# akanimax/thr3ed_atom

Measured on AMD Instinct MI355X. Metric: ray-samples/sec (fwd+bwd) training step, 800x800 images @ 128^3 SH-2 ReLU field, higher is better.
Workload: dtype f32

## Files before the change

include/relu_field.h:

```cpp
#ifndef RELU_FIELD_H_
#define RELU_FIELD_H_

#include <stdint.h>

#ifdef __cplusplus
extern "C" {
#endif

#define RF_ABI_VERSION 4
#define RF_BRICK_4X8X8 488

enum {
  RF_OK = 0,
  RF_ERR_NULL_POINTER = -1,
  RF_ERR_BAD_SHAPE = -2,
  RF_ERR_UNSUPPORTED = -3,
  RF_ERR_LAUNCH = -4
};

enum {
  RF_DENSITY_RELU = 0,
  RF_DENSITY_SOFTPLUS = 1,
  RF_DENSITY_ABS = 2,
  RF_DENSITY_IDENTITY = 3
// ... 117 lines not shown
                            int32_t* hist_dev, void* stream);
int rf_scatter_records(const RFGrid* grid, const int16_t* keys_dev, const float* records_dev, int64_t capacity,
                       int32_t* cursor_dev, int32_t render_diffuse, float* records_sorted_dev, int32_t* hist_dev, int32_t num_keys,
                       void* stream);
int rf_expand_records(const RFGrid* grid, const float* records_dev, const int64_t* perm_dev, const int64_t* begin_dev,
                      int64_t capacity, int32_t render_diffuse, float* records_sorted_dev, void* stream);

int rf_brick_accumulate(const RFGrid* grid, int32_t brick_size, const RFBrickList* lists, int32_t num_lists,
                        float* grad_densities_dev, float* grad_features_dev, int32_t accumulate, void* stream);

typedef struct RFAdamState {
  float* param_first_dev;
  float* param_second_dev;
  float* exp_avg_first_dev;
  float* exp_avg_second_dev;
  float* exp_avg_sq_first_dev;
  float* exp_avg_sq_second_dev;
  float lr, beta1, beta2, eps;
  int32_t step;
} RFAdamState;

int rf_brick_accumulate_adam(const RFGrid* grid, int32_t brick_size, const RFBrickList* lists, int32_t num_lists,
                             const RFAdamState* adam, void* stream);

int rf_brick_accumulate_adam_mirror(const RFGrid* grid, int32_t brick_size, const RFBrickList* lists, int32_t num_lists,
                                    const RFAdamState* adam, float* mirror_densities_dev, float* mirror_features_dev, void* stream);

int rf_brick_accumulate_adam_range(const RFGrid* grid, int32_t brick_size, const RFBrickList* lists, int32_t num_lists,
                                   const RFAdamState* adam, int32_t first_brick, int32_t num_bricks, void* stream);

int64_t rf_brick_split_scratch_bytes(const RFGrid* grid, int32_t num_bricks, int32_t parts);
int rf_brick_accumulate_adam_split(const RFGrid* grid, int32_t brick_size, const RFBrickList* lists, int32_t num_lists,
                                   const RFAdamState* adam, int32_t first_brick, int32_t num_bricks, int32_t parts, void* scratch_dev,
                                   int64_t scratch_bytes, void* stream);

int rf_grid_query(const RFGrid* grid, const float* points_dev, int64_t num_points, float* out_dev, void* stream);

int rf_grid_query_backward(const RFGrid* grid, const float* points_dev, int64_t num_points,
                           const float* grad_out_dev, float* grad_densities_dev, float* grad_features_dev,
                           void* stream);

int rf_build_occupancy(const RFGrid* grid, float threshold, uint32_t* occupancy_dev, void* stream);

int rf_upsample_grid(const RFGrid* src, const RFGrid* dst, void* stream);

int rf_convert_grid(const RFGrid* src, const RFGrid* dst, void* stream);
// ... 79 lines not shown
```

thr3ed_atom_amd/_lib.py:

```python
import ctypes as C
import os
import subprocess
from typing import Optional

CSRC_DIR = os.path.join(os.path.dirname(os.path.abspath(__file__)), "csrc")
INCLUDE_DIR = os.path.join(os.path.dirname(os.path.dirname(os.path.abspath(__file__))), "include")
LIB_NAME = "librelu_field_hip.so"
LIB_PATH = os.environ.get("RF_LIB_PATH") or os.path.join(CSRC_DIR, LIB_NAME)
SOURCES = ["relu_field_kernels.hip", "mesh_kernels.hip"]
HIPCC_FLAGS = ["--offload-arch=gfx950", "-O3", "-std=c++17", "-ffp-contract=off", "-fPIC", "-shared"]

ABI_VERSION = 4

DENSITY_MODES = {"relu": 0, "softplus": 1, "abs": 2, "identity": 3}
LAYOUTS = {"reference": 0, "split": 1, "bricked": 2}
FLAG_WHITE_BKGD = 1
FLAG_RENDER_DIFFUSE = 2
FLAG_AABB_SAMPLING = 4
FLAG_OCCUPANCY_SKIP = 8
FLAG_JITTER_KEYED = 16
ERR_UNSUPPORTED = -3
STEP_FORWARD = 1
STEP_EMIT = 2
STEP_BRICKS = 4
# ... 4 lines not shown
STEP_DIFFUSE_CHAIN = 128
STEP_SPECULAR_FORWARD = 256

EXPORTED_SYMBOLS = [
    "rf_abi_version",
    "rf_abi_struct_size",
    "rf_error_string",
    "rf_cast_rays",
    "rf_cast_selected_rays",
    "rf_select_rays_and_pixels",
    "rf_ray_aabb_bounds",
    "rf_render_forward",
    "rf_frame_render_kernel",
    "rf_render_backward",
    "rf_render_backward_emit",
    "rf_expand_records",
    "rf_expanded_record_floats",
    "rf_bin_offsets",
    "rf_render_backward_emit_direct",
    "rf_scatter_records",
    "rf_brick_accumulate",
    "rf_brick_accumulate_adam",
    "rf_brick_accumulate_adam_mirror",
    "rf_brick_accumulate_adam_range",
    "rf_brick_accumulate_adam_split",
    "rf_brick_split_scratch_bytes",
    "rf_grid_query",
    "rf_grid_query_backward",
    "rf_build_occupancy",
    "rf_upsample_grid",
    "rf_convert_grid",
    "rf_l1_loss_grad",
    "rf_adam_step",
    "rf_train_step",
    "rf_render_forward_pair",
    "rf_l1_loss_grad_pair",
    "rf_bin_offsets_pair",
    "rf_render_backward_emit_direct_pair",
    "rf_mesh_tiles",
    "rf_mesh_count",
    "rf_mesh_emit",
]


class RFGrid(C.Structure):
    _fields_ = [
# ... 188 lines not shown
        C.POINTER(RFRayBatch),
        u32,
        C.POINTER(RFRenderOut),
        C.POINTER(RFRenderGrads),
        vp,
        vp,
        vp,
    ]
    lib.rf_render_backward_emit.argtypes = [
        C.POINTER(RFGrid), C.POINTER(RFRayBatch), u32, C.POINTER(RFRenderOut), C.POINTER(RFRenderGrads), i32, vp, vp, vp, vp,
    ]
    lib.rf_expand_records.argtypes = [C.POINTER(RFGrid), vp, vp, vp, i64, i32, vp, vp]
    lib.rf_expanded_record_floats.argtypes = [i32]
    lib.rf_expanded_record_floats.restype = i32
    lib.rf_bin_offsets.argtypes = [vp, i32, vp, vp, vp]
    lib.rf_render_backward_emit_direct.argtypes = [
        C.POINTER(RFGrid), C.POINTER(RFRayBatch), u32, C.POINTER(RFRenderOut), C.POINTER(RFRenderGrads), i32, vp, vp, vp, vp,
    ]
    lib.rf_scatter_records.argtypes = [C.POINTER(RFGrid), vp, vp, i64, vp, i32, vp, vp, i32, vp]
    lib.rf_brick_accumulate.argtypes = [C.POINTER(RFGrid), i32, C.POINTER(RFBrickList), i32, vp, vp, i32, vp]
    lib.rf_brick_accumulate_adam.argtypes = [C.POINTER(RFGrid), i32, C.POINTER(RFBrickList), i32, C.POINTER(RFAdamState), vp]
    lib.rf_brick_accumulate_adam_range.argtypes = [C.POINTER(RFGrid), i32, C.POINTER(RFBrickList), i32, C.POINTER(RFAdamState), i32, i32, vp]
    lib.rf_brick_accumulate_adam_mirror.argtypes = [C.POINTER(RFGrid), i32, C.POINTER(RFBrickList), i32, C.POINTER(RFAdamState), vp, vp, vp]
    lib.rf_brick_accumulate_adam_split.argtypes = [C.POINTER(RFGrid), i32, C.POINTER(RFBrickList), i32, C.POINTER(RFAdamState), i32, i32, i32, vp, i64, vp]
    lib.rf_brick_split_scratch_bytes.argtypes = [C.POINTER(RFGrid), i32, i32]
    lib.rf_train_step.argtypes = [C.POINTER(RFGrid), C.POINTER(RFTrainStep), vp]
    lib.rf_grid_query.argtypes = [C.POINTER(RFGrid), vp, i64, vp, vp]
    lib.rf_grid_query_backward.argtypes = [C.POINTER(RFGrid), vp, i64, vp, vp, vp, vp]
    lib.rf_upsample_grid.argtypes = [C.POINTER(RFGrid), C.POINTER(RFGrid), vp]
    lib.rf_convert_grid.argtypes = [C.POINTER(RFGrid), C.POINTER(RFGrid), vp]
    lib.rf_build_occupancy.argtypes = [C.POINTER(RFGrid), f32, vp, vp]
    lib.rf_l1_loss_grad.argtypes = [vp, vp, i64, f32, vp, vp, vp]
    lib.rf_adam_step.argtypes = [vp, vp, vp, vp, i64, f32, f32, f32, f32, i32, i32, vp]
    lib.rf_render_forward_pair.argtypes = [C.POINTER(RFGrid), C.POINTER(RFRayBatch), C.POINTER(u32), C.POINTER(RFRenderOut), vp]
    lib.rf_l1_loss_grad_pair.argtypes = [C.POINTER(vp), vp, i64, f32, C.POINTER(vp), vp, vp, vp]
    lib.rf_bin_offsets_pair.argtypes = [C.POINTER(vp), i32, C.POINTER(vp), C.POINTER(vp), vp]
    lib.rf_render_backward_emit_direct_pair.argtypes = [C.POINTER(RFGrid), C.POINTER(RFRayBatch), C.POINTER(u32), C.POINTER(RFPassScratch), vp]
    lib.rf_mesh_tiles.argtypes = [C.POINTER(RFGrid), i32]
    lib.rf_mesh_count.argtypes = [C.POINTER(RFGrid), i32, f32, vp, vp]
    lib.rf_mesh_emit.argtypes = [C.POINTER(RFGrid), i32, f32, vp, i64, i64, vp, vp, vp, vp, vp, vp]
    for name in EXPORTED_SYMBOLS:
        if name not in ("rf_error_string",):
            getattr(lib, name).restype = C.c_int64 if name in ("rf_brick_split_scratch_bytes", "rf_mesh_tiles") else C.c_int
    if lib.rf_abi_version() != ABI_VERSION:
        raise RuntimeError(f"{LIB_PATH}: ABI version {lib.rf_abi_version()} != {ABI_VERSION} (stale build? run __graft_entry__.build())")
    lib.rf_abi_struct_size.argtypes = [C.c_int]
# ... 16 lines not shown
```

thr3ed_atom_amd/csrc/relu_field_kernels.hip:

```cpp
#include <hip/hip_runtime.h>
#include <stdint.h>

#include <atomic>
#include <cstdlib>
#include <type_traits>

#include "relu_field.h"

namespace {

#ifndef RF_FWD_WAVES
#define RF_FWD_WAVES 4
#endif
#ifndef RF_EMIT_WAVES
#define RF_EMIT_WAVES 6
#endif
#ifndef RF_EMIT_G
#define RF_EMIT_G 2
#endif
constexpr int kWave = 64;
constexpr int kWavesPerBlock = 4;
constexpr int kBlock = kWave * kWavesPerBlock;
constexpr float kInfinity = 1e10f;
constexpr float kZeroPlus = 1e-10f;
// ... 108 lines not shown
    *p = v;
  }
}
template <bool NT>
__device__ __forceinline__ float4 load_f4(const float4* p) {
  if constexpr (NT) {
    const vf4 t = __builtin_nontemporal_load(reinterpret_cast<const vf4*>(p));
    return make_float4(t[0], t[1], t[2], t[3]);
  } else {
    return *p;
  }
}
#ifndef RF_NT_RECORD_STORE
#define RF_NT_RECORD_STORE 1
#endif
#ifndef RF_NT_CACHE_STORE
#define RF_NT_CACHE_STORE 1
#endif
#ifndef RF_NT_RECORD_LOAD
#define RF_NT_RECORD_LOAD 0
#endif
#ifndef RF_NT_CACHE_LOAD
#define RF_NT_CACHE_LOAD 1
#endif

__device__ __forceinline__ void wave_lds_fence() {
  __builtin_amdgcn_fence(__ATOMIC_RELEASE, "wavefront");
  __builtin_amdgcn_wave_barrier();
  __builtin_amdgcn_fence(__ATOMIC_ACQUIRE, "wavefront");
}

template <int CTRL, int ROW_MASK>
__device__ __forceinline__ float dpp_move(float old, float src) {
  return __builtin_bit_cast(float, __builtin_amdgcn_update_dpp(__builtin_bit_cast(int, old), __builtin_bit_cast(int, src),
                                                               CTRL, ROW_MASK, 0xf, false));
}
constexpr int kDppRowShr1 = 0x111, kDppRowShr2 = 0x112, kDppRowShr4 = 0x114, kDppRowShr8 = 0x118;
constexpr int kDppRowBcast15 = 0x142, kDppRowBcast31 = 0x143, kDppWaveShr1 = 0x138, kDppWaveShl1 = 0x130;

__device__ __forceinline__ void wave_incl_scan_trans(float& e, float& a) {
  auto step = [&](auto ctrl_tag, auto mask_tag) {
    constexpr int CTRL = decltype(ctrl_tag)::value, MASK = decltype(mask_tag)::value;
    const float ep = dpp_move<CTRL, MASK>(1.0f, e), ap = dpp_move<CTRL, MASK>(0.0f, a);
    a = __builtin_fmaf(a, ep, ap);
    e = e * ep;
  };
// ... 1871 lines not shown
  const int B = ONE_ROUND ? 8 : (1 << a.shift);
  const int SY = brick_row_stride(B, C), SX = brick_slab_stride(B, C);
  const int tid = threadIdx.x;
  const bool split = g.layout == RF_LAYOUT_SPLIT;
  if (split && (C & 3) == 0 && (g.dstride & 3) == 0 && (C == 4 || (g.fstride & 3) == 0)) {
    constexpr int QN = C / 4;
    constexpr int QR = QN > 1 ? QN - 1 : 1;
    const int nq = (BX == 4 ? 4 : B) * B * B * QN;
    auto quad_of = [&](int i, int& fx, int& fy, int& fz, int& qd) -> bool {
      const int col = (i >> a.shift) / QN, r = i - col * (B * QN);
      const bool first = r < B;
      fz = first ? r : (r - B) / QR;
      qd = first ? 0 : 1 + (r - B) - fz * QR;
      fx = col >> a.shift;
      fy = col & (B - 1);
      return i < nq && X0 + fx < g.X && Y0 + fy < g.Y && Z0 + fz < g.Z;
    };
    if constexpr (ADAM) {
      constexpr int U = (QN == 7) ? 4 : 1;
      const AdamArgs& ad = a.adam;
      if constexpr (ONE_ROUND) {
        unsigned int bo[QN];
        int lds_at[QN];
        float4 p4[QN];
        vf4 m4[QN], v4[QN];
#pragma unroll
        for (int u = 0; u < QN; ++u) {
          int fx, fy, fz, qd;
          if (u == 0) {
            fx = tid >> 6;
            fy = (tid >> 3) & 7;
            fz = tid & 7;
            qd = 0;
          } else {
            const int j = (u - 1) * TH + tid, col = j / 48, r = j - col * 48;
            fz = r / 6;
            qd = 1 + r - 6 * fz;
            fx = col >> 3;
            fy = col & 7;
          }
          const bool ok = X0 + fx < g.X && Y0 + fy < g.Y && Z0 + fz < g.Z;
          const unsigned int lin = ok ? node_lin(g, X0 + fx, Y0 + fy, Z0 + fz) : 0u;
          const unsigned int o = u == 0 ? __umul24(lin, (unsigned)g.dstride) : __umul24(lin, (unsigned)g.fstride) + 4u * (unsigned)(qd - 1);
          bo[u] = ok ? o * 4u : 0xffffffffu;
          lds_at[u] = fx * SX + fy * SY + fz * CS + 4 * qd;
        }
#pragma unroll
        for (int u = 0; u < QN; ++u) {
          if (bo[u] != 0xffffffffu) {
            const char* pb = reinterpret_cast<const char*>(u == 0 ? ad.p1 : ad.p2);
            const char* mb = reinterpret_cast<const char*>(u == 0 ? ad.m1 : ad.m2);
            const char* vb = reinterpret_cast<const char*>(u == 0 ? ad.v1 : ad.v2);
            p4[u] = *reinterpret_cast<const float4*>(pb + bo[u]);
            m4[u] = __builtin_nontemporal_load(reinterpret_cast<const vf4*>(mb + bo[u]));
            v4[u] = __builtin_nontemporal_load(reinterpret_cast<const vf4*>(vb + bo[u]));
          }
        }
#pragma unroll
        for (int u = 0; u < QN; ++u) {
          if (bo[u] == 0xffffffffu) continue;
          const float4 gq = any ? *reinterpret_cast<const float4*>(&acc[lds_at[u]]) : make_float4(0.f, 0.f, 0.f, 0.f);
          float gg[4] = {gq.x, gq.y, gq.z, gq.w};
          float pn[4] = {p4[u].x, p4[u].y, p4[u].z, p4[u].w};
          if (u == 0 && g.mode == RF_DENSITY_ABS) {
            const float dv = pn[0] * g.rho;
            gg[0] = (dv > 0.f) ? gg[0] : ((dv < 0.f) ? -gg[0] : 0.0f);
          }
          vf4 mn, vn;
#pragma unroll
          for (int c = 0; c < 4; ++c) {
            float mm = m4[u][c], vv = v4[u][c];
            adam_update(pn[c], mm, vv, gg[c], ad.step, ad.b1, ad.b2, ad.eps, ad.inv_bc2_sqrt);
            mn[c] = mm;
            vn[c] = vv;
          }
          char* pb = reinterpret_cast<char*>(u == 0 ? ad.p1 : ad.p2);
          char* mb = reinterpret_cast<char*>(u == 0 ? ad.m1 : ad.m2);
          char* vb = reinterpret_cast<char*>(u == 0 ? ad.v1 : ad.v2);
          *reinterpret_cast<float4*>(pb + bo[u]) = make_float4(pn[0], pn[1], pn[2], pn[3]);
          __builtin_nontemporal_store(mn, reinterpret_cast<vf4*>(mb + bo[u]));
          __builtin_nontemporal_store(vn, reinterpret_cast<vf4*>(vb + bo[u]));
          if constexpr (MIRROR) *reinterpret_cast<float4*>(const_cast<float*>(&acc[lds_at[u]])) = make_float4(pn[0], pn[1], pn[2], pn[3]);
        }
        if constexpr (MIRROR) {
          __syncthreads();
          constexpr int F = 3 * K, FQ = 2 * F, CQ = FQ + 2;
          for (int i = tid; i < 32 * CQ; i += TH) {
            const int col = i / CQ, r = i - col * CQ;
            const int fx = col >> 3, fy = col & 7;
            const float* img = acc + fx * SX + fy * SY;
            const unsigned int lin0 = node_lin(g, X0 + fx, Y0 + fy, Z0);
            float v[4];
            if (r < FQ) {
#pragma unroll
              for (int t = 0; t < 4; ++t) {
                const int e = 4 * r + t;
                const int nz = e / F, f = e - nz * F;
                const int colour = f / K, k = f - colour * K;
                v[t] = img[nz * CS + (k == 0 ? 1 + colour : 4 + colour * (K - 1) + (k - 1))];
              }
              *reinterpret_cast<float4*>(gfeat + (size_t)(__umul24(lin0, (unsigned)F) + 4u * (unsigned)r)) = make_float4(v[0], v[1], v[2], v[3]);
            } else {
              const int z0 = 4 * (r - FQ);
#pragma unroll
              for (int t = 0; t < 4; ++t) v[t] = img[(z0 + t) * CS];
              *reinterpret_cast<float4*>(gdens + (size_t)(lin0 + (unsigned)z0)) = make_float4(v[0], v[1], v[2], v[3]);
// ... 536 lines not shown
      const unsigned long long* other = images + (long long)j * pairs;
      float2* own = reinterpret_cast<float2*>(acc);
      for (int i = tid; i < pairs; i += TH) {
        const unsigned long long o = __hip_atomic_load(other + i, __ATOMIC_RELAXED, __HIP_MEMORY_SCOPE_AGENT);
        float2 v = any ? own[i] : make_float2(0.f, 0.f);
        v.x += __uint_as_float((uint32_t)o);
        v.y += __uint_as_float((uint32_t)(o >> 32));
        own[i] = v;
      }
      any = true;
      __syncthreads();
    }
    if (tid <= parts) state[tid] = 0;
    __syncthreads();
  }
#if defined(RF_BRICK_PROFILE) || defined(RF_BRICK_ABLATE)
  if (!(a.stagger & 0x400000))
#endif
  brick_flush<K, ADAM, ONE_ROUND, TH, BX, MIRROR>(g, a, acc, any, X0, Y0, Z0, gdens, gfeat);
  RF_PROF_MARK(4);
  RF_PROF_END();
}

__device__ __forceinline__ long long channel_offset(const GridArgs& g, unsigned int lin, int ch, int K, bool& in_first) {
  if (g.layout == RF_LAYOUT_REFERENCE) {
    in_first = ch == 0;
    if (ch == 0) return (long long)lin * g.dstride;
    if (ch < 4) return (long long)lin * g.fstride + (long long)(ch - 1) * K;
    const int j = ch - 4, colour = j / (K - 1), kk = 1 + j - colour * (K - 1);
    return (long long)lin * g.fstride + (long long)colour * K + kk;
  }
  in_first = ch < 4;
  return ch < 4 ? (long long)lin * g.dstride + ch : (long long)lin * g.fstride + (ch - 4);
}

struct UpsampleAxis {
  int i0, i1;
  float w0, w1;
};
__device__ __forceinline__ UpsampleAxis upsample_axis(int dst, int in_size, float scale) {
  float src = fmaf(scale, (float)dst + 0.5f, -0.5f);
  src = src < 0.0f ? 0.0f : src;
  UpsampleAxis a;
  a.i0 = min((int)floorf(src), in_size - 1);
  a.i1 = a.i0 + (a.i0 < in_size - 1 ? 1 : 0);
  const float lambda = fminf(fmaxf(src - (float)a.i0, 0.0f), 1.0f);
// ... 1192 lines not shown
  if (diffuse) return launch_scatter<2>(keys_dev, records_dev, capacity, cursor_dev, records_sorted_dev, hist_dev, num_keys, st);
  return launch_scatter<3>(keys_dev, records_dev, capacity, cursor_dev, records_sorted_dev, hist_dev, num_keys, st);
}

int32_t rf_expanded_record_floats(int32_t num_features) { return 4 * record_quads(num_features / 3); }

extern "C++" {
template <int K, bool ADAM, bool ONE_ROUND = false, bool SPLIT = false, int BX = 8, bool MIRROR = false>
static int launch_gather(const GridArgs& g, const BrickArgs& a, int nbricks, float* gd, float* gf, hipStream_t st) {
  const int B = 1 << a.shift;
  const size_t lds = (size_t)gather_lds_words(B, 3 * K + 1, BX) * sizeof(float);
  if (lds > 150 * 1024) return RF_ERR_UNSUPPORTED;
  static std::atomic<size_t> configured[64];
  int dev = 0;
  if (hipGetDevice(&dev) != hipSuccess || dev < 0 || dev >= 64) return RF_ERR_LAUNCH;
  if (lds > configured[dev].load(std::memory_order_relaxed)) {
    if (hipFuncSetAttribute(reinterpret_cast<const void*>(&brick_gather_kernel<K, ADAM, ONE_ROUND, SPLIT, BX, MIRROR>),
                            hipFuncAttributeMaxDynamicSharedMemorySize, (int)lds) != hipSuccess)
      return RF_ERR_LAUNCH;
    configured[dev].store(lds, std::memory_order_relaxed);
  }
  hipLaunchKernelGGL((brick_gather_kernel<K, ADAM, ONE_ROUND, SPLIT, BX, MIRROR>), dim3(nbricks * (SPLIT ? a.parts : 1)), dim3(BX == 4 ? kBrickThreads / 2 : kBrickThreads), lds, st, g, a,
                     gd, gf);
  return launch_status();
}
}

static int check_fused_adam(const RFGrid* grid, const RFAdamState* adam, int K, bool base_only) {
  const int C = 3 * K + 1;
  if (grid->layout == RF_LAYOUT_REFERENCE || (C & 3) || (base_only && grid->num_features != 3)) return RF_ERR_UNSUPPORTED;
  if ((grid->density_stride & 3) || (C > 4 && (grid->feature_stride & 3))) return RF_ERR_UNSUPPORTED;
  if (!adam->param_first_dev || !adam->exp_avg_first_dev || !adam->exp_avg_sq_first_dev) return RF_ERR_NULL_POINTER;
  if (C > 4 && (!adam->param_second_dev || !adam->exp_avg_second_dev || !adam->exp_avg_sq_second_dev)) return RF_ERR_NULL_POINTER;
  if (adam->param_first_dev != grid->densities_dev || (C > 4 && adam->param_second_dev != grid->features_dev)) return RF_ERR_BAD_SHAPE;
  if (adam->step < 1) return RF_ERR_BAD_SHAPE;
  {
    unsigned long long nodes = 1;
    for (int ax = 0; ax < 3; ++ax) nodes *= (unsigned long long)((grid->dims[ax] + 7) / 8 * 8);
    const unsigned long long smax = (unsigned long long)(grid->density_stride > grid->feature_stride ? grid->density_stride : grid->feature_stride);
    if (nodes * smax >= (1ull << 31)) return RF_ERR_UNSUPPORTED;
  }
  const uintptr_t align = (uintptr_t)adam->param_first_dev | (uintptr_t)adam->exp_avg_first_dev | (uintptr_t)adam->exp_avg_sq_first_dev |
                          (C > 4 ? ((uintptr_t)adam->param_second_dev | (uintptr_t)adam->exp_avg_second_dev | (uintptr_t)adam->exp_avg_sq_second_dev) : 0);
  if (align & 15u) return RF_ERR_BAD_SHAPE;
  return RF_OK;
}
// ... 66 lines not shown
    a.adam.inv_bc2_sqrt = (float)(1.0 / sqrt(bc2));
    {
      unsigned long long nodes = 1;
      for (int ax = 0; ax < 3; ++ax) nodes *= (unsigned long long)((grid->dims[ax] + 7) / 8 * 8);
      const unsigned long long smax = (unsigned long long)(grid->density_stride > grid->feature_stride ? grid->density_stride : grid->feature_stride);
      a.adam.byte_offsets_fit_32_bits = nodes * smax < (1ull << 30) && nodes <= (1ull << 24) && smax < (1ull << 24);
    }
#if defined(RF_BRICK_PROFILE) || defined(RF_BRICK_ABLATE)
    {
      const char* e = getenv("RF_BRICK_STAGGER");
      a.stagger = e ? atoi(e) : 0;
    }
#endif
    const bool one_round = a.adam.byte_offsets_fit_32_bits && shift == 3;
    if (slab4) {
      if (!one_round || parts > 1 || (K != 1 && K != 9)) return RF_ERR_UNSUPPORTED;
      if (grad_densities_dev) {
        if (!grad_features_dev || (grid->dims[0] & 3) || (grid->dims[1] & 7) || (grid->dims[2] & 7) || g.bricked || first_brick != 0 || nbricks != nb[0] * nb[1] * nb[2])
          return RF_ERR_UNSUPPORTED;
        if ((reinterpret_cast<uintptr_t>(grad_densities_dev) | reinterpret_cast<uintptr_t>(grad_features_dev)) & 15u) return RF_ERR_BAD_SHAPE;
        return K == 1 ? launch_gather<1, true, true, false, 4, true>(g, a, nbricks, grad_densities_dev, grad_features_dev, st)
                      : launch_gather<9, true, true, false, 4, true>(g, a, nbricks, grad_densities_dev, grad_features_dev, st);
      }
      return K == 1 ? launch_gather<1, true, true, false, 4>(g, a, nbricks, nullptr, nullptr, st) : launch_gather<9, true, true, false, 4>(g, a, nbricks, nullptr, nullptr, st);
    }
    if (grad_densities_dev) return RF_ERR_UNSUPPORTED;
    if (parts > 1) {
      if (!one_round) return RF_ERR_UNSUPPORTED;
      if (parts > kMaxListsPerKind || !scratch_dev) return parts > kMaxListsPerKind ? RF_ERR_BAD_SHAPE : RF_ERR_NULL_POINTER;
      const long long words = brick_acc_words(8, 3 * K + 1);
      const long long state_bytes = ((long long)nbricks * (1 + parts) * 4 + 255) / 256 * 256;
      if (scratch_bytes < state_bytes + (long long)nbricks * parts * words * 4 || ((uintptr_t)scratch_dev & 15u)) return RF_ERR_BAD_SHAPE;
      a.parts = parts;
      a.part_state = reinterpret_cast<int*>(scratch_dev);
      a.partial = reinterpret_cast<float*>(reinterpret_cast<char*>(scratch_dev) + state_bytes);
      return K == 1 ? launch_gather<1, true, true, true>(g, a, nbricks, nullptr, nullptr, st) : launch_gather<9, true, true, true>(g, a, nbricks, nullptr, nullptr, st);
    }
    switch (K) {
      case 1:
        return one_round ? launch_gather<1, true, true>(g, a, nbricks, nullptr, nullptr, st) : launch_gather<1, true, false>(g, a, nbricks, nullptr, nullptr, st);
      default:
        return one_round ? launch_gather<9, true, true>(g, a, nbricks, nullptr, nullptr, st) : launch_gather<9, true, false>(g, a, nbricks, nullptr, nullptr, st);
    }
  }
  if (slab4) {
    if (K != 1 && K != 9) return RF_ERR_UNSUPPORTED;
    return K == 1 ? launch_gather<1, false, true, false, 4>(g, a, nbricks, grad_densities_dev, grad_features_dev, st)
                  : launch_gather<9, false, true, false, 4>(g, a, nbricks, grad_densities_dev, grad_features_dev, st);
  }
  switch (K) {
    case 1:
      return shift == 3 ? launch_gather<1, false, true>(g, a, nbricks, grad_densities_dev, grad_features_dev, st)
                        : launch_gather<1, false, false>(g, a, nbricks, grad_densities_dev, grad_features_dev, st);
    case 4:
      return shift == 3 ? launch_gather<4, false, true>(g, a, nbricks, grad_densities_dev, grad_features_dev, st)
                        : launch_gather<4, false, false>(g, a, nbricks, grad_densities_dev, grad_features_dev, st);
    case 9:
      return shift == 3 ? launch_gather<9, false, true>(g, a, nbricks, grad_densities_dev, grad_features_dev, st)
                        : launch_gather<9, false, false>(g, a, nbricks, grad_densities_dev, grad_features_dev, st);
    default:
      return shift == 3 ? launch_gather<16, false, true>(g, a, nbricks, grad_densities_dev, grad_features_dev, st)
                        : launch_gather<16, false, false>(g, a, nbricks, grad_densities_dev, grad_features_dev, st);
  }
}

int rf_brick_accumulate(const RFGrid* grid, int32_t brick_size, const RFBrickList* lists, int32_t num_lists,
                        float* grad_densities_dev, float* grad_features_dev, int32_t accumulate, void* stream) {
  return brick_accumulate_impl(grid, brick_size, lists, num_lists, grad_densities_dev, grad_features_dev, accumulate, nullptr, 0, 0, stream);
}

int rf_brick_accumulate_adam(const RFGrid* grid, int32_t brick_size, const RFBrickList* lists, int32_t num_lists,
                             const RFAdamState* adam, void* stream) {
  if (!adam) return RF_ERR_NULL_POINTER;
  return brick_accumulate_impl(grid, brick_size, lists, num_lists, nullptr, nullptr, 0, adam, 0, 0, stream);
}

int rf_brick_accumulate_adam_mirror(const RFGrid* grid, int32_t brick_size, const RFBrickList* lists, int32_t num_lists,
                                    const RFAdamState* adam, float* mirror_densities_dev, float* mirror_features_dev, void* stream) {
  if (!adam || !mirror_densities_dev || !mirror_features_dev) return RF_ERR_NULL_POINTER;
  if (brick_size != RF_BRICK_4X8X8) return RF_ERR_UNSUPPORTED;
  return brick_accumulate_impl(grid, brick_size, lists, num_lists, mirror_densities_dev, mirror_features_dev, 0, adam, 0, 0, stream);
}

int rf_brick_accumulate_adam_range(const RFGrid* grid, int32_t brick_size, const RFBrickList* lists, int32_t num_lists,
                                   const RFAdamState* adam, int32_t first_brick, int32_t num_bricks, void* stream) {
  if (!adam) return RF_ERR_NULL_POINTER;
// ... 377 lines not shown
```

Baseline: 16.04 billion.

## Add warp-specialized brick pipeline kernel and batch Adam stores after loads

Adds a persistent warp-specialized brick kernel in which producer waves stage records into double-buffered LDS, matrix waves accumulate per-brick gradients, and Adam waves prefetch parameters and apply updates, all coordinated by LDS flag counters with a poll timeout and an error symbol. The aim is to overlap record fetching, accumulation and the optimizer update across bricks. This path is off unless RF_BRICK_PIPELINE is set. The existing one-round Adam path is also reordered so every load is issued before any store, with stores flushed afterwards, meant to keep loads from being serialized behind stores at the cost of more live registers.

```diff
diff --git a/include/relu_field.h b/include/relu_field.h
--- a/include/relu_field.h
+++ b/include/relu_field.h
@@ -163,6 +163,8 @@
 
 int rf_brick_accumulate_adam(const RFGrid* grid, int32_t brick_size, const RFBrickList* lists, int32_t num_lists,
                              const RFAdamState* adam, void* stream);
+
+int rf_brick_pipeline_error(int32_t reset);
 
 int rf_brick_accumulate_adam_mirror(const RFGrid* grid, int32_t brick_size, const RFBrickList* lists, int32_t num_lists,
                                     const RFAdamState* adam, float* mirror_densities_dev, float* mirror_features_dev, void* stream);
diff --git a/thr3ed_atom_amd/_lib.py b/thr3ed_atom_amd/_lib.py
--- a/thr3ed_atom_amd/_lib.py
+++ b/thr3ed_atom_amd/_lib.py
@@ -50,6 +50,7 @@
     "rf_brick_accumulate",
     "rf_brick_accumulate_adam",
     "rf_brick_accumulate_adam_mirror",
+    "rf_brick_pipeline_error",
     "rf_brick_accumulate_adam_range",
     "rf_brick_accumulate_adam_split",
     "rf_brick_split_scratch_bytes",
@@ -284,6 +285,7 @@
     lib.rf_brick_accumulate_adam.argtypes = [C.POINTER(RFGrid), i32, C.POINTER(RFBrickList), i32, C.POINTER(RFAdamState), vp]
     lib.rf_brick_accumulate_adam_range.argtypes = [C.POINTER(RFGrid), i32, C.POINTER(RFBrickList), i32, C.POINTER(RFAdamState), i32, i32, vp]
     lib.rf_brick_accumulate_adam_mirror.argtypes = [C.POINTER(RFGrid), i32, C.POINTER(RFBrickList), i32, C.POINTER(RFAdamState), vp, vp, vp]
+    lib.rf_brick_pipeline_error.argtypes = [i32]
     lib.rf_brick_accumulate_adam_split.argtypes = [C.POINTER(RFGrid), i32, C.POINTER(RFBrickList), i32, C.POINTER(RFAdamState), i32, i32, i32, vp, i64, vp]
     lib.rf_brick_split_scratch_bytes.argtypes = [C.POINTER(RFGrid), i32, i32]
     lib.rf_train_step.argtypes = [C.POINTER(RFGrid), C.POINTER(RFTrainStep), vp]
diff --git a/thr3ed_atom_amd/csrc/relu_field_kernels.hip b/thr3ed_atom_amd/csrc/relu_field_kernels.hip
--- a/thr3ed_atom_amd/csrc/relu_field_kernels.hip
+++ b/thr3ed_atom_amd/csrc/relu_field_kernels.hip
@@ -154,6 +154,9 @@
 #endif
 #ifndef RF_NT_CACHE_LOAD
 #define RF_NT_CACHE_LOAD 1
+#endif
+#ifndef RF_FLUSH_STORES_AFTER_LOADS
+#define RF_FLUSH_STORES_AFTER_LOADS 1
 #endif
 
 __device__ __forceinline__ void wave_lds_fence() {
@@ -2071,8 +2074,16 @@
       if constexpr (ONE_ROUND) {
         unsigned int bo[QN];
         int lds_at[QN];
-        float4 p4[QN];
-        vf4 m4[QN], v4[QN];
+        vf4 p4[QN], m4[QN], v4[QN];
+        auto flush_store = [&](int u) {
+          char* pb = reinterpret_cast<char*>(u == 0 ? ad.p1 : ad.p2);
+          char* mb = reinterpret_cast<char*>(u == 0 ? ad.m1 : ad.m2);
+          char* vb = reinterpret_cast<char*>(u == 0 ? ad.v1 : ad.v2);
+          *reinterpret_cast<vf4*>(pb + bo[u]) = p4[u];
+          __builtin_nontemporal_store(m4[u], reinterpret_cast<vf4*>(mb + bo[u]));
+          __builtin_nontemporal_store(v4[u], reinterpret_cast<vf4*>(vb + bo[u]));
+          if constexpr (MIRROR) *reinterpret_cast<vf4*>(const_cast<float*>(&acc[lds_at[u]])) = p4[u];
+        };
 #pragma unroll
         for (int u = 0; u < QN; ++u) {
           int fx, fy, fz, qd;
@@ -2100,37 +2111,42 @@
             const char* pb = reinterpret_cast<const char*>(u == 0 ? ad.p1 : ad.p2);
             const char* mb = reinterpret_cast<const char*>(u == 0 ? ad.m1 : ad.m2);
             const char* vb = reinterpret_cast<const char*>(u == 0 ? ad.v1 : ad.v2);
-            p4[u] = *reinterpret_cast<const float4*>(pb + bo[u]);
+            p4[u] = *reinterpret_cast<const vf4*>(pb + bo[u]);
             m4[u] = __builtin_nontemporal_load(reinterpret_cast<const vf4*>(mb + bo[u]));
             v4[u] = __builtin_nontemporal_load(reinterpret_cast<const vf4*>(vb + bo[u]));
           }
         }
+#if RF_FLUSH_STORES_AFTER_LOADS
+#pragma unroll
+        for (int u = 0; u < QN; ++u) asm volatile("" : "+v"(p4[u]), "+v"(m4[u]), "+v"(v4[u]));
+#endif
 #pragma unroll
         for (int u = 0; u < QN; ++u) {
           if (bo[u] == 0xffffffffu) continue;
           const float4 gq = any ? *reinterpret_cast<const float4*>(&acc[lds_at[u]]) : make_float4(0.f, 0.f, 0.f, 0.f);
           float gg[4] = {gq.x, gq.y, gq.z, gq.w};
-          float pn[4] = {p4[u].x, p4[u].y, p4[u].z, p4[u].w};
+          float pn[4] = {p4[u][0], p4[u][1], p4[u][2], p4[u][3]};
           if (u == 0 && g.mode == RF_DENSITY_ABS) {
             const float dv = pn[0] * g.rho;
             gg[0] = (dv > 0.f) ? gg[0] : ((dv < 0.f) ? -gg[0] : 0.0f);
           }
-          vf4 mn, vn;
 #pragma unroll
           for (int c = 0; c < 4; ++c) {
             float mm = m4[u][c], vv = v4[u][c];
             adam_update(pn[c], mm, vv, gg[c], ad.step, ad.b1, ad.b2, ad.eps, ad.inv_bc2_sqrt);
-            mn[c] = mm;
-            vn[c] = vv;
+            m4[u][c] = mm;
+            v4[u][c] = vv;
           }
-          char* pb = reinterpret_cast<char*>(u == 0 ? ad.p1 : ad.p2);
-          char* mb = reinterpret_cast<char*>(u == 0 ? ad.m1 : ad.m2);
-          char* vb = reinterpret_cast<char*>(u == 0 ? ad.v1 : ad.v2);
-          *reinterpret_cast<float4*>(pb + bo[u]) = make_float4(pn[0], pn[1], pn[2], pn[3]);
-          __builtin_nontemporal_store(mn, reinterpret_cast<vf4*>(mb + bo[u]));
-          __builtin_nontemporal_store(vn, reinterpret_cast<vf4*>(vb + bo[u]));
-          if constexpr (MIRROR) *reinterpret_cast<float4*>(const_cast<float*>(&acc[lds_at[u]])) = make_float4(pn[0], pn[1], pn[2], pn[3]);
+          p4[u] = vf4{pn[0], pn[1], pn[2], pn[3]};
+#if !RF_FLUSH_STORES_AFTER_LOADS
+          flush_store(u);
+#endif
         }
+#if RF_FLUSH_STORES_AFTER_LOADS
+#pragma unroll
+        for (int u = 0; u < QN; ++u)
+          if (bo[u] != 0xffffffffu) flush_store(u);
+#endif
         if constexpr (MIRROR) {
           __syncthreads();
           constexpr int F = 3 * K, FQ = 2 * F, CQ = FQ + 2;
@@ -2713,6 +2729,509 @@
   RF_PROF_END();
 }
 
+#ifndef RF_PIPE_POLL_LIMIT
+#define RF_PIPE_POLL_LIMIT (1 << 22)
+#endif
+__device__ int g_brick_pipeline_error;
+
+struct PipeState {
+  int sbar;
+  int full[2], freed[2];
+  int ifull[2], ifreed[2];
+  int meta[2];
+  int abort;
+};
+
+__device__ __forceinline__ bool pipe_wait(PipeState& ps, int* word, int target) {
+  for (int n = 0;; ++n) {
+    const int v = __builtin_amdgcn_readfirstlane(__hip_atomic_load(word, __ATOMIC_RELAXED, __HIP_MEMORY_SCOPE_WORKGROUP));
+    if (v >= target) break;
+    if (__builtin_amdgcn_readfirstlane(__hip_atomic_load(&ps.abort, __ATOMIC_RELAXED, __HIP_MEMORY_SCOPE_WORKGROUP))) return false;
+    if (n >= RF_PIPE_POLL_LIMIT) {
+      if ((threadIdx.x & (kWave - 1)) == 0) {
+        __hip_atomic_store(&ps.abort, 1, __ATOMIC_RELAXED, __HIP_MEMORY_SCOPE_WORKGROUP);
+        atomicOr(&g_brick_pipeline_error, 1);
+      }
+      return false;
+    }
+    __builtin_amdgcn_s_sleep(1);
+  }
+  asm volatile("" ::: "memory");
+  return true;
+}
+__device__ __forceinline__ void pipe_signal(int* word) {
+  asm volatile("s_waitcnt lgkmcnt(0)" ::: "memory");
+  if ((threadIdx.x & (kWave - 1)) == 0) __hip_atomic_fetch_add(word, 1, __ATOMIC_RELAXED, __HIP_MEMORY_SCOPE_WORKGROUP);
+}
+
+constexpr int kPipeThreads = 1024;
+template <int K>
+__host__ __device__ constexpr int pipe_stage_words() { return (kGatherBatch / 2) * gather_record_words((3 * K + 1 + 3) / 4 * 4) + (kGatherBatch / 2 + 4) * kGatherWtab; }
+template <int K>
+__host__ __device__ inline int pipe_image_words() { return 4 * brick_slab_stride(8, 3 * K + 1) + 64; }
+template <int K>
+__host__ __device__ inline int pipe_lds_words() { return 2 * pipe_stage_words<K>() + 2 * pipe_image_words<K>(); }
+
+template <int K>
+__global__ __launch_bounds__(kPipeThreads) void brick_pipeline_kernel(GridArgs g, BrickArgs a, int nbricks, int stride) {
+  constexpr int GB = kGatherBatch / 2;
+  constexpr int GROW = GB + 4;
+  constexpr int C = 3 * K + 1;
+  constexpr int C4 = (C + 3) / 4 * 4;
+  constexpr int QW = record_quads(K);
+  constexpr int QN = record_quads(1);
+  constexpr int NT = (C4 + 15) / 16;
+  static_assert(NT == 1 || NT == 2, "SH degree 0 or 2");
+  constexpr int CS = C4;
+  constexpr int NW = GB / 64;
+  constexpr int NWV = 8;
+  constexpr int B = 8, npz = 2, npy = 4, ntiles = 16;
+  constexpr int SW = pipe_stage_words<K>();
+  const int SY = brick_row_stride(B, C), SX = brick_slab_stride(B, C);
+  const int IW = pipe_image_words<K>();
+  extern __shared__ __attribute__((aligned(16))) float lds[];
+  __shared__ uint32_t s_tmask[2][GB];
+  __shared__ unsigned char s_list[ntiles][GB + 24];
+  __shared__ __attribute__((aligned(16))) int s_wstart[kMaxRangesKind], s_wcum[kMaxRangesKind + 8];
+  __shared__ __attribute__((aligned(16))) int s_nstart[kMaxRangesKind], s_ncum[kMaxRangesKind + 8];
+  __shared__ int s_part[4];
+  __shared__ PipeState ps;
+
+  const int tid = threadIdx.x;
+  const int lane = tid & (kWave - 1);
+  const int wave = tid >> 6;
+  for (int s = 0; s < 2; ++s) {
+    float4* wt = reinterpret_cast<float4*>(lds + s * SW + GB * gather_record_words(C4));
+    for (int i = tid; i < GROW * kGatherWtab / 4; i += kPipeThreads) wt[i] = make_float4(0.f, 0.f, 0.f, 0.f);
+  }
+  if (tid < (int)(sizeof(PipeState) / sizeof(int))) reinterpret_cast<int*>(&ps)[tid] = 0;
+  __syncthreads();
+
+  auto brick_origin = [&](int bl, int& bx, int& by, int& bz) {
+    const int brick = a.brick_first + bl;
+    bz = brick % a.nbz;
+    by = (brick / a.nbz) % a.nby;
+    bx = brick / (a.nbz * a.nby);
+  };
+
+  if (wave < 4) {
+    const int rec_id = tid & (GB - 1);
+    const int half = tid >= GB;
+    int sgen = 0;
+    auto sbar = [&]() -> bool {
+      ++sgen;
+      pipe_signal(&ps.sbar);
+      return pipe_wait(ps, &ps.sbar, 4 * sgen);
+    };
+    uint32_t wprev0 = 0x00ffffffu, wprev1 = 0x00ffffffu;
+    int q = 0;
+    for (int j = 0;; ++j) {
+      const int bl = blockIdx.x + j * stride;
+      if (bl >= nbricks) break;
+      int bx, by, bz;
+      brick_origin(bl, bx, by, bz);
+      const int X0 = bx << 2, Y0 = by << 3, Z0 = bz << 3;
+      if (!sbar()) return;
+      {
+        const int kind = tid >> 7, i = tid & 127;
+        int start = 0, cnt = 0;
+        if (i < kRangeEntries && (kind ? a.nnarrow : a.nwide) > 0)
+          brick_range_entry(a, kind ? a.narrow[0].offsets : a.wide[0].offsets, bx, by, bz, i, start, cnt);
+        int cum = cnt;
+#pragma unroll
+        for (int d = 1; d < kWave; d <<= 1) {
+          const int up = __shfl_up(cum, d);
+          if (lane >= d) cum += up;
+        }
+        if (lane == kWave - 1) s_part[wave] = cum;
+        if (!sbar()) return;
+        if (wave & 1) cum += s_part[wave - 1];
+        int* st_ = kind ? s_nstart : s_wstart;
+        int* cu_ = kind ? s_ncum : s_wcum;
+        if (i < kMaxRangesKind) {
+          st_[i] = start;
+          cu_[i + 1] = cum;
+        }
+        if (i == 0) cu_[0] = 0;
+        if (!sbar()) return;
+      }
+      const int total = s_wcum[kMaxRangesKind];
+      const int total_d = s_ncum[kMaxRangesKind];
+      const int nba = (total + GB - 1) / GB, nbd = (total_d + GB - 1) / GB;
+
+      auto acquire_slot = [&]() -> bool { return pipe_wait(ps, &ps.freed[q & 1], NWV * (q >> 1)); };
+      auto publish = [&](int nrec, int wide, int last) {
+        const int sl = q & 1;
+        if (tid == 0) ps.meta[sl] = nrec | (wide << 8) | (last << 9);
+        pipe_signal(&ps.full[sl]);
+        ++q;
+      };
+      if (nba + nbd == 0) {
+        if (!acquire_slot()) return;
+        publish(0, 0, 1);
+        continue;
+      }
+
+      auto stage = [&](auto expand_tag, float4 q0, float4 q1, float4 q2, int nrec) {
+        constexpr bool EXPAND = decltype(expand_tag)::value;
+        constexpr int RW = gather_record_words(EXPAND ? C4 : 4);
+        const int sl = q & 1;
+        float* rows = lds + sl * SW;
+        float* wtab = rows + GB * gather_record_words(C4);
+        if (half == 0) {
+          uint32_t& wprev = sl ? wprev1 : wprev0;
+          uint32_t tm = 0, wnow = 0x00ffffffu;
+          float* wcol = wtab + rec_id;
+#pragma unroll
+          for (int ax = 0; ax < 3; ++ax) {
+            const int c1 = (int)((wprev >> (8 * ax)) & 0xffu);
+            if (c1 != 0xff) {
+              if (c1 >= 1) wcol[(ax * 8 + c1 - 1) * GROW] = 0.0f;
+              if (c1 < (ax == 0 ? 4 : B)) wcol[(ax * 8 + c1) * GROW] = 0.0f;
+            }
+          }
+          if (rec_id < nrec) {
+            const float idx[3] = {q0.x, q0.y, q0.z};
+            const int org[3] = {X0, Y0, Z0};
+            uint32_t pb[3];
+            wnow = 0;
+#pragma unroll
+            for (int ax = 0; ax < 3; ++ax) {
+              const float fl = floorf(idx[ax]);
+              const int c = (int)fl - org[ax];
+              const int sh = ax == 2 ? 2 : 1;
+              uint32_t bits = 0;
+              if (c >= 0) {
+                wcol[(ax * 8 + c) * GROW] = (fl + 1.0f) - idx[ax];
+                bits |= 1u << (c >> sh);
+              }
+              if (c + 1 < (ax == 0 ? 4 : B)) {
+                wcol[(ax * 8 + c + 1) * GROW] = idx[ax] - fl;
+                bits |= 1u << ((c + 1) >> sh);
+              }
+              pb[ax] = bits;
+              wnow |= (uint32_t)(c + 1) << (8 * ax);
+            }
+            uint32_t yz = 0;
+#pragma unroll
+            for (int py = 0; py < 4; ++py)
+              if ((pb[1] >> py) & 1u) yz |= pb[2] << (py * npz);
+#pragma unroll
+            for (int px = 0; px < 4; ++px)
+              if ((pb[0] >> px) & 1u) tm |= yz << (px * npy * npz);
+          }
+          wprev = wnow;
+          s_tmask[sl][rec_id] = tm;
+        }
+        float* row = rows + rec_id * RW;
+        if constexpr (EXPAND) {
+          const float graw[3] = {q1.x, q1.y, q1.z};
+          constexpr int NQ = C4 / 4;
+          if (half == 0) {
+            *reinterpret_cast<float4*>(row) = make_float4(q0.w, graw[0] * kC0, graw[1] * kC0, graw[2] * kC0);
+          } else {
+            float Y[16];
+            sh_basis<K>(q1.w, q2.x, q2.y, Y);
+#pragma unroll
+            for (int qq = 1; qq < NQ; ++qq) {
+              float v[4];
+#pragma unroll
+              for (int x = 0; x < 4; ++x) v[x] = (4 * qq + x < C) ? record_channel<K>(4 * qq + x, q0.w, graw, Y) : 0.0f;
+              *reinterpret_cast<float4*>(row + 4 * qq) = make_float4(v[0], v[1], v[2], v[3]);
+            }
+          }
+        } else {
+          if (half == 0) *reinterpret_cast<float4*>(row) = q1;
+        }
+      };
+      using Yes = std::integral_constant<bool, true>;
+      using No = std::integral_constant<bool, false>;
+      int sri = 0, dri = 0, rlo = 0, rhi = 0, dlo = 0, dhi = 0;
+      const float4* rptr = a.wide[0].rec;
+      const float4* dptr = a.narrow[0].rec;
+      float4 w0 = make_float4(0.f, 0.f, 0.f, 0.f), w1 = w0, w2 = w0, d0 = w0, d1 = w0;
+      auto range_of = [&](const int* cum, int v) -> int {
+        const int4* c4 = reinterpret_cast<const int4*>(cum);
+        const int4 c0 = c4[0], c1 = c4[1], c2 = c4[2], c3 = c4[3];
+        return (c0.y <= v) + (c0.z <= v) + (c0.w <= v) + (c1.x <= v) + (c1.y <= v) + (c1.z <= v) + (c1.w <= v) + (c2.x <= v) + (c2.y <= v) + (c2.z <= v) +
+               (c2.w <= v) + (c3.x <= v) + (c3.y <= v) + (c3.z <= v);
+      };
+      auto fetch_wide = [&](int s) {
+        const int nrec = min(GB, total - s * GB);
+        const int v = s * GB + min(rec_id, nrec - 1);
+        if (v < rlo || v >= rhi) {
+          sri = range_of(s_wcum, v);
+          rlo = s_wcum[sri];
+          rhi = s_wcum[sri + 1];
+          rptr = a.wide[0].rec + (long long)(s_wstart[sri] - rlo) * QW;
+        }
+        const float4* p = rptr + (long long)v * QW;
+        w0 = load_f4<RF_NT_RECORD_LOAD>(p);
+        w1 = load_f4<RF_NT_RECORD_LOAD>(p + 1);
+        if constexpr (QW > 2) w2 = load_f4<RF_NT_RECORD_LOAD>(p + 2);
+      };
+      auto fetch_narrow = [&](int sd) {
+        const int nrec = min(GB, total_d - sd * GB);
+        const int v = sd * GB + min(rec_id, nrec - 1);
+        if (v < dlo || v >= dhi) {
+          dri = range_of(s_ncum, v);
+          dlo = s_ncum[dri];
+          dhi = s_ncum[dri + 1];
+          dptr = a.narrow[0].rec + (long long)(s_nstart[dri] - dlo) * QN;
+        }
+        const float4* p = dptr + (long long)v * QN;
+        d0 = load_f4<RF_NT_RECORD_LOAD>(p);
+        d1 = load_f4<RF_NT_RECORD_LOAD>(p + 1);
+      };
+      if (nbd > 0) fetch_narrow(0);
+      if (nba > 0) fetch_wide(0);
+      for (int s = 0; s < nba; ++s) {
+        const int nrec = min(GB, total - s * GB);
+        if (!acquire_slot()) return;
+        if constexpr (K > 1)
+          stage(Yes{}, w0, w1, w2, nrec);
+        else
+          stage(No{}, w0, w1, w2, nrec);
+        fetch_wide(min(s + 1, nba - 1));
+        publish(nrec, 1, (s + 1 == nba && nbd == 0) ? 1 : 0);
+      }
+      for (int sd = 0; sd < nbd; ++sd) {
+        const int nrec = min(GB, total_d - sd * GB);
+        if (!acquire_slot()) return;
+        stage(No{}, d0, d1, d1, nrec);
+        fetch_narrow(min(sd + 1, nbd - 1));
+        publish(nrec, 0, sd + 1 == nbd ? 1 : 0);
+      }
+    }
+    return;
+  }
+
+  if (wave < 4 + NWV) {
+    const int mw = wave - 4;
+    const int mi = lane & 15;
+    const int mdx = mi >> 3, mdy = (mi >> 2) & 1, mdz = mi & 3;
+    const int kk = lane >> 4;
+    const int jj = lane & 15;
+    f32x4 accr[2][NT];
+#pragma unroll
+    for (int tl = 0; tl < 2; ++tl)
+#pragma unroll
+      for (int nt = 0; nt < NT; ++nt) accr[tl][nt] = f32x4{0.f, 0.f, 0.f, 0.f};
+
+    auto process = [&](auto wide_tag, int sl, int nrec) {
+      constexpr bool WIDE = decltype(wide_tag)::value;
+      constexpr int RW = gather_record_words(WIDE ? C4 : 4);
+      constexpr int NTW = WIDE ? NT : 1;
+      const float* rows = lds + sl * SW;
+      const float* wtab = rows + GB * gather_record_words(C4);
+      int cnt[2] = {0, 0};
+#pragma unroll
+      for (int wd = 0; wd < NW; ++wd) {
+        if (wd * 64 >= nrec) break;
+        const uint32_t tmv = s_tmask[sl][wd * 64 + lane] >> mw;
+#pragma unroll
+        for (int tl = 0; tl < 2; ++tl) {
+          const bool hit = (tmv >> (NWV * tl)) & 1u;
+          const unsigned long long m = __ballot(hit);
+          const int pos = cnt[tl] + __builtin_amdgcn_mbcnt_hi((uint32_t)(m >> 32), __builtin_amdgcn_mbcnt_lo((uint32_t)m, 0));
+          if (hit) s_list[tl * NWV + mw][pos] = (unsigned char)(wd * 64 + lane);
+          cnt[tl] += __popcll(m);
+        }
+      }
+#pragma unroll
+      for (int tl = 0; tl < 2; ++tl)
+        if (lane < 8) s_list[tl * NWV + mw][cnt[tl] + lane] = 0;
+#pragma unroll
+      for (int tl = 0; tl < 2; ++tl) {
+        const int t = tl * NWV + mw;
+        const int n = cnt[tl];
+        if (n > 0) {
+          const int pz = t % npz, py = (t / npz) % npy, px = t / (npz * npy);
+          const float* wx = wtab + (2 * px + mdx) * GROW;
+          const float* wy = wtab + (8 + 2 * py + mdy) * GROW;
+          const float* wz = wtab + (16 + 4 * pz + mdz) * GROW;
+          const float* gbase = rows + (WIDE ? jj : (jj & 3));
+          const uint32_t a_list = lds_offset(s_list[t]) + kk;
+          const uint32_t a_x = lds_offset(wx), a_y = lds_offset(wy), a_z = lds_offset(wz), a_g = lds_offset(gbase);
+          const int nq = (n + 3) >> 2;
+          uint32_t ra = 0, rb = 0;
+          float aw0 = 0.f, aw1 = 0.f, aw2 = 0.f, bw0 = 0.f, bw1 = 0.f, bw2 = 0.f;
+          float ag0 = 0.f, ag1 = 0.f, bg0 = 0.f, bg1 = 0.f;
+          auto request_ops = [&](float& w0, float& w1, float& w2, float& g0, float& g1, uint32_t r) {
+            lds_request_f32<0>(w0, a_x + 4 * r);
+            lds_request_f32<0>(w1, a_y + 4 * r);
+            lds_request_f32<0>(w2, a_z + 4 * r);
+            const uint32_t a_row = a_g + (uint32_t)__umul24(r, RW * 4);
+            lds_request_f32<0>(g0, a_row);
+            if constexpr (NTW > 1) lds_request_f32<64>(g1, a_row);
+          };
+          auto wait_ops = [&](float& w0, float& w1, float& w2, float& g0, float& g1, uint32_t& r) { lds_wait(w0, w1, w2, g0, g1, r); };
+          auto multiply = [&](float w0, float w1, float w2, float g0, float g1, int qi) {
+            const float wv = (w0 * w1) * w2;
+            const float wa = (4 * qi + kk < n) ? wv : 0.0f;
+            const float ga = (WIDE || jj < 4) ? g0 : 0.0f;
+            accr[tl][0] = __builtin_amdgcn_mfma_f32_16x16x4f32(wa, ga, accr[tl][0], 0, 0, 0);
+            if constexpr (NTW > 1) accr[tl][1] = __builtin_amdgcn_mfma_f32_16x16x4f32(wa, g1, accr[tl][1], 0, 0, 0);
+          };
+          lds_request_u8(ra, a_list);
+          lds_request_u8(rb, a_list + 4);
+          lds_wait(ra, rb);
+          request_ops(aw0, aw1, aw2, ag0, ag1, ra);
+          for (int qi = 0; qi < nq; qi += 2) {
+            wait_ops(aw0, aw1, aw2, ag0, ag1, rb);
+            lds_request_u8(ra, a_list + 4 * qi + 8);
+            request_ops(bw0, bw1, bw2, bg0, bg1, rb);
+            multiply(aw0, aw1, aw2, ag0, ag1, qi);
+            if (qi + 1 < nq) {
+              wait_ops(bw0, bw1, bw2, bg0, bg1, ra);
+              lds_request_u8(rb, a_list + 4 * qi + 12);
+              request_ops(aw0, aw1, aw2, ag0, ag1, ra);
+              multiply(bw0, bw1, bw2, bg0, bg1, qi + 1);
+            }
+          }
+          wait_ops(aw0, aw1, aw2, ag0, ag1, ra);
+          wait_ops(bw0, bw1, bw2, bg0, bg1, rb);
+        }
+      }
+    };
+    using Yes = std::integral_constant<bool, true>;
+    using No = std::integral_constant<bool, false>;
+    int q = 0;
+    for (int j = 0;; ++j) {
+      const int bl = blockIdx.x + j * stride;
+      if (bl >= nbricks) break;
+      for (;;) {
+        const int sl = q & 1;
+        if (!pipe_wait(ps, &ps.full[sl], 4 * ((q >> 1) + 1))) return;
+        const int meta = __builtin_amdgcn_readfirstlane(ps.meta[sl]);
+        const int nrec = meta & 0xff;
+        if (nrec > 0) {
+          if (meta & 0x100)
+            process(Yes{}, sl, nrec);
+          else
+            process(No{}, sl, nrec);
+        }
+        pipe_signal(&ps.freed[sl]);
+        ++q;
+        if (meta & 0x200) break;
+      }
+      const int il = j & 1;
+      if (!pipe_wait(ps, &ps.ifreed[il], 4 * (j >> 1))) return;
+      float* img = lds + 2 * SW + il * IW;
+#pragma unroll
+      for (int tl = 0; tl < 2; ++tl) {
+        const int t = tl * NWV + mw;
+        const int pz = t % npz, py = (t / npz) % npy, px = t / (npz * npy);
+#pragma unroll
+        for (int nt = 0; nt < NT; ++nt) {
+          const int ch = 16 * nt + jj;
+#pragma unroll
+          for (int e = 0; e < 4; ++e) {
+            const int i = 4 * kk + e;
+            const int nx = 2 * px + (i >> 3), ny = 2 * py + ((i >> 2) & 1), nz = 4 * pz + (i & 3);
+            if (ch < CS) img[nx * SX + ny * SY + nz * CS + ch] = accr[tl][nt][e];
+          }
+          accr[tl][nt] = f32x4{0.f, 0.f, 0.f, 0.f};
+        }
+      }
+      pipe_signal(&ps.ifull[il]);
+    }
+    return;
+  }
+
+  {
+    constexpr int TH = 256;
+    constexpr int QF = C / 4;
+    const AdamArgs& ad = a.adam;
+    for (int j = 0;; ++j) {
+      const int bl = blockIdx.x + j * stride;
+      if (bl >= nbricks) break;
+      int ft;
+      asm volatile("v_mov_b32 %0, %1" : "=v"(ft) : "v"(tid - (4 + NWV) * kWave));
+      int bx, by, bz;
+      brick_origin(bl, bx, by, bz);
+      const int X0 = bx << 2, Y0 = by << 3, Z0 = bz << 3;
+      auto quad_of = [&](int u, int& fx, int& fy, int& fz, int& qd) {
+        if (u == 0) {
+          fx = ft >> 6;
+          fy = (ft >> 3) & 7;
+          fz = ft & 7;
+          qd = 0;
+        } else {
+          const int jq = (u - 1) * TH + ft, col = jq / 48, r = jq - col * 48;
+          fz = r / 6;
+          qd = 1 + r - 6 * fz;
+          fx = col >> 3;
+          fy = col & 7;
+        }
+      };
+      unsigned int bo[QF];
+      vf4 p4[QF];
+      vf4 m4[QF], v4[QF];
+#pragma unroll
+      for (int u = 0; u < QF; ++u) {
+        int fx, fy, fz, qd;
+        quad_of(u, fx, fy, fz, qd);
+        const bool ok = X0 + fx < g.X && Y0 + fy < g.Y && Z0 + fz < g.Z;
+        const unsigned int lin = ok ? node_lin(g, X0 + fx, Y0 + fy, Z0 + fz) : 0u;
+        const unsigned int o = u == 0 ? __umul24(lin, (unsigned)g.dstride) : __umul24(lin, (unsigned)g.fstride) + 4u * (unsigned)(qd - 1);
+        bo[u] = ok ? o * 4u : 0xffffffffu;
+      }
+#pragma unroll
+      for (int u = 0; u < QF; ++u) {
+        if (bo[u] != 0xffffffffu) {
+          const char* pb = reinterpret_cast<const char*>(u == 0 ? ad.p1 : ad.p2);
+          const char* mb = reinterpret_cast<const char*>(u == 0 ? ad.m1 : ad.m2);
+          const char* vb = reinterpret_cast<const char*>(u == 0 ? ad.v1 : ad.v2);
+          p4[u] = *reinterpret_cast<const vf4*>(pb + bo[u]);
+          m4[u] = __builtin_nontemporal_load(reinterpret_cast<const vf4*>(mb + bo[u]));
+          v4[u] = __builtin_nontemporal_load(reinterpret_cast<const vf4*>(vb + bo[u]));
+        }
+      }
+      const int il = j & 1;
+      if (!pipe_wait(ps, &ps.ifull[il], NWV * ((j >> 1) + 1))) return;
+      const float* img = lds + 2 * SW + il * IW;
+      float step = ad.step, b1 = ad.b1, b2 = ad.b2, eps = ad.eps, ibc = ad.inv_bc2_sqrt;
+      asm volatile("" : "+s"(step), "+s"(b1), "+s"(b2), "+s"(eps), "+s"(ibc));
+      asm volatile("v_mov_b32 %0, %0" : "+v"(ft));
+#pragma unroll
+      for (int u = 0; u < QF; ++u) asm volatile("" : "+v"(p4[u]), "+v"(m4[u]), "+v"(v4[u]));
+#pragma unroll
+      for (int u = 0; u < QF; ++u) {
+        if (bo[u] == 0xffffffffu) continue;
+        int fx, fy, fz, qd;
+        quad_of(u, fx, fy, fz, qd);
+        const float4 gq = *reinterpret_cast<const float4*>(&img[fx * SX + fy * SY + fz * CS + 4 * qd]);
+        float gg[4] = {gq.x, gq.y, gq.z, gq.w};
+        float pn[4] = {p4[u][0], p4[u][1], p4[u][2], p4[u][3]};
+        if (u == 0 && g.mode == RF_DENSITY_ABS) {
+          const float dv = pn[0] * g.rho;
+          gg[0] = (dv > 0.f) ? gg[0] : ((dv < 0.f) ? -gg[0] : 0.0f);
+        }
+#pragma unroll
+        for (int c = 0; c < 4; ++c) {
+          float mm = m4[u][c], vv = v4[u][c];
+          adam_update(pn[c], mm, vv, gg[c], step, b1, b2, eps, ibc);
+          m4[u][c] = mm;
+          v4[u][c] = vv;
+        }
+        p4[u] = vf4{pn[0], pn[1], pn[2], pn[3]};
+      }
+#pragma unroll
+      for (int u = 0; u < QF; ++u) {
+        if (bo[u] == 0xffffffffu) continue;
+        char* pb = reinterpret_cast<char*>(u == 0 ? ad.p1 : ad.p2);
+        char* mb = reinterpret_cast<char*>(u == 0 ? ad.m1 : ad.m2);
+        char* vb = reinterpret_cast<char*>(u == 0 ? ad.v1 : ad.v2);
+        *reinterpret_cast<vf4*>(pb + bo[u]) = p4[u];
+        __builtin_nontemporal_store(m4[u], reinterpret_cast<vf4*>(mb + bo[u]));
+        __builtin_nontemporal_store(v4[u], reinterpret_cast<vf4*>(vb + bo[u]));
+      }
+      pipe_signal(&ps.ifreed[il]);
+    }
+  }
+}
+
 __device__ __forceinline__ long long channel_offset(const GridArgs& g, unsigned int lin, int ch, int K, bool& in_first) {
   if (g.layout == RF_LAYOUT_REFERENCE) {
     in_first = ch == 0;
@@ -3951,6 +4470,27 @@
   }
   hipLaunchKernelGGL((brick_gather_kernel<K, ADAM, ONE_ROUND, SPLIT, BX, MIRROR>), dim3(nbricks * (SPLIT ? a.parts : 1)), dim3(BX == 4 ? kBrickThreads / 2 : kBrickThreads), lds, st, g, a,
                      gd, gf);
+  return launch_status();
+}
+
+template <int K>
+static int launch_pipeline(const GridArgs& g, const BrickArgs& a, int nbricks, hipStream_t st) {
+  const size_t lds = (size_t)pipe_lds_words<K>() * sizeof(float);
+  static std::atomic<size_t> configured[64];
+  int dev = 0;
+  if (hipGetDevice(&dev) != hipSuccess || dev < 0 || dev >= 64) return RF_ERR_LAUNCH;
+  if (lds > configured[dev].load(std::memory_order_relaxed)) {
+    if (hipFuncSetAttribute(reinterpret_cast<const void*>(&brick_pipeline_kernel<K>), hipFuncAttributeMaxDynamicSharedMemorySize, (int)lds) != hipSuccess)
+      return RF_ERR_LAUNCH;
+    configured[dev].store(lds, std::memory_order_relaxed);
+  }
+  static const int per = [] {
+    const char* e = getenv("RF_BRICK_PIPELINE_BRICKS");
+    const int v = e ? atoi(e) : 0;
+    return v > 0 ? v : 8;
+  }();
+  const int stride = ((nbricks + per - 1) / per + 7) / 8 * 8;
+  hipLaunchKernelGGL((brick_pipeline_kernel<K>), dim3(stride), dim3(kPipeThreads), lds, st, g, a, nbricks, stride);
   return launch_status();
 }
 }
@@ -4063,6 +4603,12 @@
         return K == 1 ? launch_gather<1, true, true, false, 4, true>(g, a, nbricks, grad_densities_dev, grad_features_dev, st)
                       : launch_gather<9, true, true, false, 4, true>(g, a, nbricks, grad_densities_dev, grad_features_dev, st);
       }
+      static const bool pipeline = [] {
+        const char* e = getenv("RF_BRICK_PIPELINE");
+        return e ? atoi(e) != 0 : false;
+      }();
+      if (pipeline && a.nwide <= 1 && a.nnarrow <= 1)
+        return K == 1 ? launch_pipeline<1>(g, a, nbricks, st) : launch_pipeline<9>(g, a, nbricks, st);
       return K == 1 ? launch_gather<1, true, true, false, 4>(g, a, nbricks, nullptr, nullptr, st) : launch_gather<9, true, true, false, 4>(g, a, nbricks, nullptr, nullptr, st);
     }
     if (grad_densities_dev) return RF_ERR_UNSUPPORTED;
@@ -4103,6 +4649,16 @@
       return shift == 3 ? launch_gather<16, false, true>(g, a, nbricks, grad_densities_dev, grad_features_dev, st)
                         : launch_gather<16, false, false>(g, a, nbricks, grad_densities_dev, grad_features_dev, st);
   }
+}
+
+int rf_brick_pipeline_error(int32_t reset) {
+  int v = 0;
+  if (hipMemcpyFromSymbol(&v, HIP_SYMBOL(g_brick_pipeline_error), sizeof(int)) != hipSuccess) return RF_ERR_LAUNCH;
+  if (reset) {
+    const int zero = 0;
+    if (hipMemcpyToSymbol(HIP_SYMBOL(g_brick_pipeline_error), &zero, sizeof(int)) != hipSuccess) return RF_ERR_LAUNCH;
+  }
+  return v;
 }
 
 int rf_brick_accumulate(const RFGrid* grid, int32_t brick_size, const RFBrickList* lists, int32_t num_lists,
```

Measured after the change: 16.21 billion (median of 6 runs). 1.1% higher.
